# PJLab-ADG/neuralsim

Measured on AMD Instinct MI355X. Metric: training rays/sec (fwd+bwd) NeuS 800x800, higher is better.
Workload: dtype fp16

## Files before the change

### neuralsim_amd/csrc/field.hip

```cpp
#ifndef NSIM_SCATTER_SCAN_EXIT
#define NSIM_SCATTER_SCAN_EXIT 1
#endif
#include "lotd_dev.h"
#include "mfma_mlp.h"
#include "occ_dev.h"
#include <stdlib.h>

enum { M_W1 = 0, M_W2, M_W2T, M_W1T, M_R1, M_R2, M_R3, M_R3T, M_R2T, M_R1T, M_COUNT };
enum { V_B1 = 0, V_B2, V_WH, V_RB1, V_RB2, V_RB3, V_SCAL, V_COUNT };

struct FieldLayout {
  int64_t mat[M_COUNT];
  int64_t vec[V_COUNT];
  int64_t total;
  int elt;
  int split;
};

static const int kMatUo[M_COUNT] = {64, 64, 64, 32, 64, 64, 32, 64, 64, 32};
static const int kMatUi[M_COUNT] = {32, 64, 64, 64, 32, 64, 64, 32, 64, 64};

static inline int mat_uo(int m, int nc) { return m == M_W1T ? 32 * nc : kMatUo[m]; }
static inline int mat_ui(int m, int nc) { return m == M_W1 ? 32 * nc : kMatUi[m]; }
static inline int field_nc(int num_levels) { return num_levels > 16 ? 2 : 1; }
static inline int field_ne(const NsimFieldMeta* meta) { return meta->embed_E > 0 ? 2 : 0; }
static inline int field_ni(const NsimFieldMeta* meta) { return field_nc(meta->lotd.num_levels) + field_ne(meta); }

static inline FieldLayout field_layout(int precision, int nc = 1) {
  FieldLayout L;
  L.elt = precision == 0 ? 2 : 4;
  L.split = precision == 2 ? 1 : 0;
  int64_t off = 0;
  for (int m = 0; m < M_COUNT; ++m) {
    L.mat[m] = off;
    off += (int64_t)mat_uo(m, nc) * mat_ui(m, nc) * L.elt;
  }
  for (int v = 0; v < V_COUNT; ++v) {
    L.vec[v] = off;
    off += 64 * 4;
  }
  L.total = off;
  return L;
}

struct SrcOff {
  int w1, w2, wh, b1, b2, bh;
  int r1, r2, r3, rb1, rb2, rb3;
  int n_sdf_w, n_sdf_b, n_rad_w, n_rad_b;
};
__host__ __device__ inline SrcOff src_off(int D, int F1 = 32) {
  SrcOff o;
  o.w1 = 0;
  o.w2 = 64 * F1;
  o.wh = (D == 2) ? 64 * F1 + 4096 : 64 * F1;
  o.n_sdf_w = o.wh + 64;
  o.b1 = 0;
  o.b2 = 64;
  o.bh = (D == 2) ? 128 : 64;
  o.n_sdf_b = o.bh + 1;
  o.r1 = 0;
  o.r2 = 64 * 26;
  o.r3 = 64 * 26 + 4096;
  o.n_rad_w = o.r3 + 192;
  o.rb1 = 0;
  o.rb2 = 64;
  o.rb3 = 128;
  o.n_rad_b = 131;
  return o;
}


#define SPLIT_LO_SCALE 2048.0f
__device__ __forceinline__ float f16_sat(float v) { return fminf(fmaxf(v, -65504.0f), 65504.0f); }
__device__ __forceinline__ void split_f16(float v, f16& hi, f16& lo) {
  v = f16_sat(v);
  hi = (f16)v;
// ... 52 lines not shown
        ((f16*)(wpack + L.mat[m]))[k] = whi;
        if (L.split) ((f16*)(wpack + L.mat[m]))[cnt + k] = (f16)((w - (float)whi) * SPLIT_LO_SCALE);
      } else {
        const int lane = (int)(k & 63);
        const int fr = (int)(k >> 6);
        const int r = fr & 15, fm = fr >> 4;
        const int nMi = Ui / 32;
        const int mo = fm / nMi, mi = fm % nMi;
        row = 32 * mo + (lane & 31);
        col = unit_of(mi, r, lane >> 5);
        ((float*)(wpack + L.mat[m]))[k] = pack_src(m, row, col, D, F1, dims.E, dims.EB, sdf_w, rad_w);
      }
      return;
    }
    base += cnt;
  }
  const int64_t vtid = tid - base;
  if (vtid >= 0 && vtid < (int64_t)V_COUNT * 64) {
    const int v = (int)(vtid >> 6), k = (int)(vtid & 63);
    const int hi = k >> 5, m = (k >> 4) & 1, r = k & 15;
    const int u = unit_of(m, r, hi);
    const SrcOff o = src_off(D, F1 + dims.E);
    float val = 0.f;
    switch (v) {
      case V_B1: val = sdf_b[o.b1 + u]; break;
      case V_B2: val = D == 2 ? sdf_b[o.b2 + u] : 0.f; break;
      case V_WH: val = sdf_w[o.wh + u]; break;
      case V_RB1: val = rad_b[o.rb1 + u]; break;
      case V_RB2: val = rad_b[o.rb2 + u]; break;
      case V_RB3: val = (u < 3) ? rad_b[o.rb3 + u] : 0.f; break;
      case V_SCAL: val = (k == 0) ? sdf_b[o.bh] : 0.f; break;
    }
    ((float*)(wpack + L.vec[v]))[k] = val;
  }
}

__global__ void __launch_bounds__(256) k_field_pack(FieldLayout L, PackDims dims, int D, int F1, const float* __restrict__ sdf_w,
                                                     const float* __restrict__ sdf_b, const float* __restrict__ rad_w,
                                                     const float* __restrict__ rad_b, char* __restrict__ wpack) {
  field_pack_elem(L, dims, D, F1, sdf_w, sdf_b, rad_w, rad_b, wpack, (int64_t)blockIdx.x * blockDim.x + threadIdx.x);
}

struct PackTwo {
  FieldLayout L[2];
  PackDims dims[2];
  char* out[2];
};
__global__ void __launch_bounds__(256) k_field_pack2(PackTwo p, int D, int F1, const float* __restrict__ sdf_w,
                                                      const float* __restrict__ sdf_b, const float* __restrict__ rad_w,
                                                      const float* __restrict__ rad_b) {
  const int64_t tid = (int64_t)blockIdx.x * blockDim.x + threadIdx.x;
  if (blockIdx.y == 0) field_pack_elem(p.L[0], p.dims[0], D, F1, sdf_w, sdf_b, rad_w, rad_b, p.out[0], tid);
  else field_pack_elem(p.L[1], p.dims[1], D, F1, sdf_w, sdf_b, rad_w, rad_b, p.out[1], tid);
}

#define NSIM_LOG2E 1.4426950408889634f
#define NSIM_LN2 0.6931471805599453f
__device__ __forceinline__ float softplus_exact(float z, float beta, float inv_beta) {
  const float t = nsim_exp2(-fabsf(z) * (beta * NSIM_LOG2E));
  return fmaxf(z, 0.f) + nsim_log2(1.0f + t) * (inv_beta * NSIM_LN2);
}
#ifdef NSIM_PROBE_CHEAP_ACT
__device__ __forceinline__ float softplus_b(float z, float beta, float inv_beta) {
  const float q = fmaxf(0.f, 1.0f - 0.25f * beta * fabsf(z));
  return fmaxf(z, 0.f) + q * q * (inv_beta * NSIM_LN2);
}
// ... 128 lines not shown
__device__ long long g_ktime1[3][64 * 24];
__device__ long long g_kiter[3][64 * 32];
#define KT(K, i)                                                                                          \
  if (blockIdx.x < 64 && wave == 0 && lane == 0) {                                                        \
    if ((i) == 0 && grp >= 0 && (grp - (int64_t)blockIdx.x) / (int64_t)gridDim.x < 32)                    \
      g_kiter[K][blockIdx.x * 32 + (grp - (int64_t)blockIdx.x) / (int64_t)gridDim.x] =                   \
          (long long)__builtin_amdgcn_s_memtime();                                                        \
    if (grp == (int64_t)blockIdx.x + gridDim.x || (i) >= 20)                                              \
      g_ktime[K][blockIdx.x * 24 + (i)] = (long long)__builtin_amdgcn_s_memtime();                        \
    else if (grp == (int64_t)blockIdx.x)                                                                  \
      g_ktime1[K][blockIdx.x * 24 + (i)] = (long long)__builtin_amdgcn_s_memtime();                       \
  }
extern "C" int nsim_debug_ktime(long long* out) {
  return (int)hipMemcpyFromSymbol(out, HIP_SYMBOL(g_ktime), sizeof(g_ktime));
}
extern "C" int nsim_debug_kiter(long long* out) {
  return (int)hipMemcpyFromSymbol(out, HIP_SYMBOL(g_kiter), sizeof(g_kiter));
}
extern "C" int nsim_debug_ktime1(long long* out) {
  return (int)hipMemcpyFromSymbol(out, HIP_SYMBOL(g_ktime1), sizeof(g_ktime1));
}
#else
#define KT(K, i)
#endif

template <int PREC>
__device__ __forceinline__ const char* stage_weights(char* smem, const FieldArgs& a, int first, int count,
                                                     FieldLayout& Lk, int& lds_used) {
  Lk = a.lay;
  nsim_prefetch_own_code(a.code_pf, smem);
  if constexpr (PREC != 1) {
    const int64_t m0 = a.lay.mat[first];
    const int64_t m1 = (first + count < M_COUNT) ? a.lay.mat[first + count] : a.lay.vec[0];
    const int64_t mbytes = m1 - m0, vbytes = a.lay.total - a.lay.vec[0];
    const f16x8* src = reinterpret_cast<const f16x8*>(a.wpack + m0);
    f16x8* dst = reinterpret_cast<f16x8*>(smem);
    for (int i = threadIdx.x; i < (int)(mbytes >> 4); i += blockDim.x) dst[i] = src[i];
    const f16x8* vsrc = reinterpret_cast<const f16x8*>(a.wpack + a.lay.vec[0]);
    f16x8* vdst = reinterpret_cast<f16x8*>(smem + mbytes);
    for (int i = threadIdx.x; i < (int)(vbytes >> 4); i += blockDim.x) vdst[i] = vsrc[i];
    for (int m = 0; m < M_COUNT; ++m) Lk.mat[m] = a.lay.mat[m] - m0;
    for (int v = 0; v < V_COUNT; ++v) Lk.vec[v] = mbytes + (a.lay.vec[v] - a.lay.vec[0]);
    lds_used = (int)((mbytes + vbytes + 15) & ~15);
    __syncthreads();
    return smem;
  } else {
    lds_used = 0;
    return a.wpack;
  }
}

__device__ __forceinline__ float vecf(const char* W, const FieldLayout& L, int v, int hi, int k) {
  return reinterpret_cast<const float*>(W + L.vec[v])[hi * 32 + k];
}

struct alignas(8) nsim_f2 { float x, y; };
template <class T>
struct alignas(2 * sizeof(T)) JPair;
template <class T>
__device__ __forceinline__ void jload6(const T* p, float (&a)[3], float (&b)[3]);
template <class T>
struct alignas(2 * sizeof(T)) JPair {
  T x, y;
};
template <class T>
__device__ __forceinline__ void jstore6(T* p, const float (&a)[3], const float (&b)[3]) {
  JPair<T>* q = reinterpret_cast<JPair<T>*>(p);
// ... 1038 lines not shown
#pragma unroll
      for (int q = 0; q < 4; ++q)
#pragma unroll
        for (int b = 0; b < 2; ++b) {
          const int l = 16 * m + 4 * q + 2 * hi + b, r0 = 16 * m + 4 * q + 2 * b;
          if (!LV_OK(l)) continue;
          float* dp = a.dh_pl + ((int64_t)l * a.S + s) * 2;
          dp[0] = dh[r0];
          dp[1] = dh[r0 + 1];
        }
    }
    KT(1, 16);
    KT(1, 17);
  }
  { const int64_t grp = -1; KT(1, 21); }
  const int F1 = 2 * a.lotd.num_levels, FIN = F1 + (NE ? a.embed_E : 0);
  const SrcOff so = src_off(SDF_D, FIN);
  const int64_t ro = (int64_t)(blockIdx.x & (unsigned)a.rep_mask) * a.rep_stride;
  auto flush_w1 = [&](int mo, int no, const f32x16& acc) {
    if (no < NC) jflush_tile(a.dsdf_w + ro + so.w1, FIN, 64, F1, mo, no, acc);
    else jflush_tile(a.dsdf_w + ro + so.w1 + (F1 - 32 * NC), FIN, 64, 32 * NC + a.embed_E, mo, no, acc);
  };
#pragma unroll
  for (int q = 0; q < NPAIR; ++q) flush_w1(wave >> 1, 2 * q + (wave & 1), accW1[q]);
  if constexpr (NODD) flush_w1(wave & 1, NI - 1, accW1[NPAIR]);
  if constexpr (SDF_D == 2) {
    jflush_tile(a.dsdf_w + ro + so.w2, 64, 64, 64, wave >> 1, wave & 1, accW2);
    if (bs2 != 0.f) atomicAdd(&a.dsdf_b[ro + so.b2 + lane], bs2);
  }
  if (bs1 != 0.f) atomicAdd(&a.dsdf_b[ro + so.b1 + lane], bs1);
  if (bsh != 0.f) atomicAdd(&a.dsdf_w[ro + so.wh + lane], bsh);
  if (lane == 0 && bh != 0.f) atomicAdd(&a.dsdf_b[ro + so.bh], bh);
  { const int64_t grp = -1; KT(1, 22); }
}

#define SDF_H_SCALE 1024.0f
#ifndef NSIM_SDF_MIN_WAVES
#define NSIM_SDF_MIN_WAVES 2
#endif
#ifndef NSIM_SDF_NBUF
#define NSIM_SDF_NBUF 1
#endif
#ifndef GLM_PTS
#define GLM_PTS 2
#endif
#ifndef GLM_PTS_WJ
#define GLM_PTS_WJ 1
#endif
#ifndef NSIM_GATHER_WJ_WAVES
#define NSIM_GATHER_WJ_WAVES 1
#endif
#ifndef NSIM_GATHER_SLOTS_WJ
#define NSIM_GATHER_SLOTS_WJ 1
#endif
#ifndef NSIM_GATHER_SLOTS
#define NSIM_GATHER_SLOTS 0
#endif
template <int PREC, bool WJ>
__global__ void __launch_bounds__(64, WJ ? NSIM_GATHER_WJ_WAVES : 1) k_lotd_gather_lm(FieldArgs a) {
  using JT = typename JPlane<PREC>::T;
  constexpr int NP = WJ ? GLM_PTS_WJ : GLM_PTS;
  const int lane = nsim_lane();
  const int xcd = (int)(blockIdx.x & 7u);
  const int64_t s0 = (int64_t)(blockIdx.x >> 3) * (64 * NP) + lane;
  int64_t Sv = a.S;
  if (a.S_dev) {
// ... 822 lines not shown
        g_grad_scratch[i].floats >= (int64_t)R * n)
      return g_grad_scratch[i].buf;
  return nullptr;
}

static void grad_scratch_fold(float* sc, int R, int64_t n_w, int64_t n_b, float* dst_w, float* dst_b, hipStream_t stream) {
  const int64_t n = n_w + n_b;
  hipLaunchKernelGGL(k_rep_reduce, dim3(nsim_blocks(n, 256)), dim3(256), 0, stream, sc, R, n, n_w, dst_w, dst_b, n);
}

static FieldArgs field_args(const NsimFieldMeta* meta) {
  FieldArgs a = FieldArgs();
  a.lotd = lotd_dev(&meta->lotd);
  a.lay = field_layout(meta->precision, field_ni(meta));
  a.embed_E = meta->embed_E;
  a.beta = meta->softplus_beta > 0.f ? meta->softplus_beta : 1e30f;
  static const int code_pf = getenv("NSIM_CODE_PREFETCH") ? atoi(getenv("NSIM_CODE_PREFETCH")) : 0;
  a.code_pf = code_pf;
  return a;
}

static unsigned field_grid(int64_t S, int64_t max_blocks, int waves = FIELD_WAVES) {
  const int64_t tiles = (S + 31) / 32;
  int64_t b = (tiles + waves - 1) / waves;
  if (b > max_blocks) b = max_blocks;
  if (b < 1) b = 1;
  return (unsigned)b;
}

static size_t weights_lds_bytes(const NsimFieldMeta* meta, int first = 0, int count = M_COUNT) {
  if (meta->precision == 1) return 0;
  const FieldLayout L = field_layout(meta->precision, field_ni(meta));
  const int64_t m1 = (first + count < M_COUNT) ? L.mat[first + count] : L.vec[0];
  return (size_t)(((m1 - L.mat[first]) + (L.total - L.vec[0]) + 15) & ~15);
}
static size_t stage_bytes(const NsimFieldMeta* meta) {
  return meta->precision == 0 ? stage_bytes_per_wave<0>() : stage_bytes_per_wave<1>();
}

static int field_waves(const NsimFieldMeta* meta, int mode) {
  return (mode == 2 && meta->precision == 0 && field_nc(meta->lotd.num_levels) == 2) ? 3 : FIELD_WAVES;
}

template <int MODE>
static int field_launch(const NsimFieldMeta* meta, const FieldArgs& a, size_t shmem, int64_t max_blocks,
                        hipStream_t stream, bool gl2 = false) {
  const int nw = field_waves(meta, MODE);
  const dim3 grid(field_grid(a.S, max_blocks, nw)), block(64 * nw);
  const int key = meta->precision * 2 + (meta->sdf_D - 1);
  if (field_ne(meta)) {
    if constexpr (MODE == 3) {
      switch ((field_nc(meta->lotd.num_levels) - 1) * 4 + key) {
        case 0: hipLaunchKernelGGL((k_field<0, 1, 3, 1, false, 2>), grid, block, shmem, stream, a); break;
        case 1: hipLaunchKernelGGL((k_field<0, 2, 3, 1, false, 2>), grid, block, shmem, stream, a); break;
        case 2: hipLaunchKernelGGL((k_field<1, 1, 3, 1, false, 2>), grid, block, shmem, stream, a); break;
        case 3: hipLaunchKernelGGL((k_field<1, 2, 3, 1, false, 2>), grid, block, shmem, stream, a); break;
        case 4: hipLaunchKernelGGL((k_field<0, 1, 3, 2, false, 2>), grid, block, shmem, stream, a); break;
        case 5: hipLaunchKernelGGL((k_field<0, 2, 3, 2, false, 2>), grid, block, shmem, stream, a); break;
        case 6: hipLaunchKernelGGL((k_field<1, 1, 3, 2, false, 2>), grid, block, shmem, stream, a); break;
        case 7: hipLaunchKernelGGL((k_field<1, 2, 3, 2, false, 2>), grid, block, shmem, stream, a); break;
      }
      NSIM_CHECK_LAUNCH();
      return 0;
    } else {
      return 36;
    }
  }
// ... 29 lines not shown
  return 0;
}

static int bwd_ablate() {
  const char* ab = getenv("NSIM_ABLATE");
  return ab ? atoi(ab) : 0;
}

#define FIELD_GRID_FWD 1024
#define FIELD_GRID_BWD 256

extern "C" {

int64_t nsim_field_wpack_bytes(const NsimFieldMeta* meta) {
  if (field_meta_check(meta)) return -1;
  return field_layout(meta->precision, field_ni(meta)).total;
}

int nsim_field_pack_weights(const NsimFieldMeta* meta, const float* sdf_w, const float* sdf_b, const float* rad_w,
                            const float* rad_b, void* wpack, void* stream) {
  const int rc = field_meta_check(meta);
  if (rc) return rc;
  const int nc = field_ni(meta);
  const FieldLayout L = field_layout(meta->precision, nc);
  PackDims dims;
  dims.E = meta->embed_E;
  dims.EB = 32 * field_nc(meta->lotd.num_levels);
  int64_t total = 0;
  for (int m = 0; m < M_COUNT; ++m) {
    dims.uo[m] = mat_uo(m, nc);
    dims.ui[m] = mat_ui(m, nc);
    total += (int64_t)dims.uo[m] * dims.ui[m];
  }
  total += (int64_t)V_COUNT * 64;
  hipLaunchKernelGGL(k_field_pack, dim3(nsim_blocks(total, 256)), dim3(256), 0, (hipStream_t)stream, L, dims,
                     meta->sdf_D, 2 * meta->lotd.num_levels, sdf_w, sdf_b, rad_w, rad_b, (char*)wpack);
  NSIM_CHECK_LAUNCH();
  return 0;
}

int nsim_jplane_elem_bytes(const NsimFieldMeta* meta) { return meta ? NSIM_J_ELEM_BYTES(meta->precision) : 0; }

int nsim_field_pack_weights2(const NsimFieldMeta* meta_a, void* wpack_a, const NsimFieldMeta* meta_b, void* wpack_b,
                             const float* sdf_w, const float* sdf_b, const float* rad_w, const float* rad_b, void* stream) {
  int rc = field_meta_check(meta_a);
  if (rc) return rc;
  rc = field_meta_check(meta_b);
  if (rc) return rc;
  if (meta_a->sdf_D != meta_b->sdf_D || meta_a->lotd.num_levels != meta_b->lotd.num_levels || meta_a->embed_E != meta_b->embed_E) return 2;
  if (!wpack_a || !wpack_b) return 4;
  const int nc = field_ni(meta_a);
  PackTwo p;
  const NsimFieldMeta* ms[2] = {meta_a, meta_b};
  int64_t most = 0;
  for (int q = 0; q < 2; ++q) {
    p.L[q] = field_layout(ms[q]->precision, nc);
    int64_t total = (int64_t)V_COUNT * 64;
    p.dims[q].E = meta_a->embed_E;
    p.dims[q].EB = 32 * field_nc(meta_a->lotd.num_levels);
    for (int m = 0; m < M_COUNT; ++m) {
      p.dims[q].uo[m] = mat_uo(m, nc);
      p.dims[q].ui[m] = mat_ui(m, nc);
      total += (int64_t)p.dims[q].uo[m] * p.dims[q].ui[m];
    }
    most = total > most ? total : most;
  }
  p.out[0] = (char*)wpack_a;
  p.out[1] = (char*)wpack_b;
  hipLaunchKernelGGL(k_field_pack2, dim3(nsim_blocks(most, 256), 2), dim3(256), 0, (hipStream_t)stream, p, meta_a->sdf_D,
                     2 * meta_a->lotd.num_levels, sdf_w, sdf_b, rad_w, rad_b);
  NSIM_CHECK_LAUNCH();
  return 0;
}

static void deal_levels(const NsimFieldMeta* meta, FieldArgs& a) {
  const int NL = field_nc(meta->lotd.num_levels) == 2 ? ((meta->lotd.num_levels + 7) & ~7) : 16;
  float cost[32], load[8] = {0, 0, 0, 0, 0, 0, 0, 0}, total = 0.f;
  bool used[32] = {false};
  for (int l = 0; l < NL; ++l) {
    cost[l] = l >= meta->lotd.num_levels ? (NL > 16 ? 0.05f : 0.35f) : (meta->lotd.type[l] == NSIM_LOTD_HASH ? 1.0f : 0.35f);
    total += cost[l];
  }
  const float limit = total / 8.0f * 1.08f;
  for (int xc = 0; xc < 8; ++xc) a.glm_n[xc] = 0;
  auto least = [&]() {
    int tx = 0;
    for (int xc = 1; xc < 8; ++xc)
      if (load[xc] < load[tx]) tx = xc;
    return tx;
  };
  auto put = [&](int xc, int l, int half, float c) {
    a.glm_lv[xc][(int)a.glm_n[xc]] = (signed char)l;
    a.glm_half[xc][(int)a.glm_n[xc]++] = (signed char)half;
    load[xc] += c;
  };
  auto tsize = [&](int l) { return l < meta->lotd.num_levels ? meta->lotd.size[l] : 0u; };
  for (int it = 0; it < NL; ++it) {
// ... 241 lines not shown
struct BwdPos {
  const float *x, *rays_o, *rays_d, *t;
  const int64_t* ridx;
};
static int field_bwd_sdf(const NsimFieldMeta* meta, const void* wpack, const BwdPos* pos, const float* h_planes,
                         const void* J_planes, int64_t S, const float* dsdf, const float* gn, float* dh_planes, float* g_planes,
                         float* dsdf_w, float* dsdf_b, float* dx, int64_t plane_pitch, void* stream) {
  const int rc = field_meta_check_full(meta);
  if (rc) return rc;
  if (S <= 0) return 0;
  if (!dsdf_w || !dsdf_b) return 26;
  if (!h_planes || !J_planes) return 28;
  if ((dh_planes != nullptr) != (g_planes != nullptr)) return 28;
  const int ne = field_ne(meta);
  if ((ne != 0) != (pos != nullptr)) return 36;
  if (ne && dx) return 36;
  FieldArgs a = field_args(meta);
  a.wpack = (const char*)wpack;
  if (pos) {
    if (!pos->x && !(pos->rays_o && pos->rays_d && pos->t && pos->ridx)) return 24;
    a.x = pos->x; a.rays_o = pos->rays_o; a.rays_d = pos->rays_d; a.t = pos->t; a.ridx = pos->ridx;
  }
  a.S = S;
  if (plane_pitch != 0 && (plane_pitch < S || (plane_pitch & 31))) return 28;
  a.PS = plane_pitch ? plane_pitch : NSIM_PLANE_PITCH(S);
  a.dsdf = dsdf; a.dnablas = gn;
  a.h_pl = const_cast<float*>(h_planes); a.J_pl = const_cast<void*>(J_planes);
  a.dh_pl = dh_planes; a.g_pl = g_planes;
  a.dsdf_w = dsdf_w; a.dsdf_b = dsdf_b;
  a.dx = dx;
  a.ablate = bwd_ablate();
  const int nc = field_nc(meta->lotd.num_levels), nw = field_waves(meta, 2);
  const char* oldp = getenv("NSIM_SDF_BWD_OLD");
  if (ne || !(oldp && atoi(oldp) == 1)) {
    const size_t row = meta->precision == 0 ? jstage_row_bytes<0>() : jstage_row_bytes<1>();
    const int ni = nc + ne;
    const bool dbuf = NSIM_BWD_DBUF && meta->precision == 0 && !ne && (nc == 2 || NSIM_BWD_JDIRECT);
    const size_t shmem = weights_lds_bytes(meta, 0, 4) + (dbuf ? 2 : 1) * (128 + (ni > 2 ? 32 * ni : 64)) * row +
                         (meta->precision == 0 && nc == 1 && !ne ? (size_t)JOINT_WAVES * (NSIM_BWD_JDIRECT ? 4096 : 16384) : 0);
    const int64_t tiles = (S + 31) / 32;
    int64_t nb = (tiles + JOINT_WAVES - 1) / JOINT_WAVES;
    const char* gcap = getenv("NSIM_SDF_BWD_GRID");
    const int64_t cap = gcap ? atoi(gcap) : 256;
    nb = nb > cap ? cap : (nb < 1 ? 1 : nb);
    const dim3 grid((unsigned)nb), block(64 * JOINT_WAVES);
    const SrcOff so = src_off(meta->sdf_D, 2 * meta->lotd.num_levels + meta->embed_E);
    int R = 1;
    float* sc = nb >= grad_replicas_min_wg() ? grad_scratch(stream, so.n_sdf_w + so.n_sdf_b, R) : nullptr;
    if (sc) {
      a.dsdf_w = sc; a.dsdf_b = sc + so.n_sdf_w;
      a.rep_mask = R - 1; a.rep_stride = so.n_sdf_w + so.n_sdf_b;
    }
    switch ((ne ? 8 : 0) + (nc - 1) * 4 + meta->precision * 2 + (meta->sdf_D - 1)) {
      case 8: hipLaunchKernelGGL((k_field_bwd_j<0, 1, 1, 2>), grid, block, shmem, (hipStream_t)stream, a); break;
      case 9: hipLaunchKernelGGL((k_field_bwd_j<0, 2, 1, 2>), grid, block, shmem, (hipStream_t)stream, a); break;
      case 10: hipLaunchKernelGGL((k_field_bwd_j<1, 1, 1, 2>), grid, block, shmem, (hipStream_t)stream, a); break;
      case 11: hipLaunchKernelGGL((k_field_bwd_j<1, 2, 1, 2>), grid, block, shmem, (hipStream_t)stream, a); break;
      case 12: hipLaunchKernelGGL((k_field_bwd_j<0, 1, 2, 2>), grid, block, shmem, (hipStream_t)stream, a); break;
      case 13: hipLaunchKernelGGL((k_field_bwd_j<0, 2, 2, 2>), grid, block, shmem, (hipStream_t)stream, a); break;
      case 14: hipLaunchKernelGGL((k_field_bwd_j<1, 1, 2, 2>), grid, block, shmem, (hipStream_t)stream, a); break;
      case 15: hipLaunchKernelGGL((k_field_bwd_j<1, 2, 2, 2>), grid, block, shmem, (hipStream_t)stream, a); break;
      case 0: hipLaunchKernelGGL((k_field_bwd_j<0, 1>), grid, block, shmem, (hipStream_t)stream, a); break;
      case 1: hipLaunchKernelGGL((k_field_bwd_j<0, 2>), grid, block, shmem, (hipStream_t)stream, a); break;
      case 2: hipLaunchKernelGGL((k_field_bwd_j<1, 1>), grid, block, shmem, (hipStream_t)stream, a); break;
      case 3: hipLaunchKernelGGL((k_field_bwd_j<1, 2>), grid, block, shmem, (hipStream_t)stream, a); break;
      case 4: hipLaunchKernelGGL((k_field_bwd_j<0, 1, 2>), grid, block, shmem, (hipStream_t)stream, a); break;
      case 5: hipLaunchKernelGGL((k_field_bwd_j<0, 2, 2>), grid, block, shmem, (hipStream_t)stream, a); break;
// ... 112 lines not shown
```

### neuralsim_amd/csrc/mfma_mlp.h

```cpp
#pragma once
#include "nsim_common.h"

__device__ __forceinline__ int unit_of(int m, int r, int hi) { return 32 * m + (r & 3) + 8 * (r >> 2) + 4 * hi; }


__device__ __forceinline__ f32x16 zero16() {
  f32x16 z;
#pragma unroll
  for (int r = 0; r < 16; ++r) z[r] = 0.f;
  return z;
}

template <int PREC, int N>
__device__ __forceinline__ float dyn_scale(const float (&v)[N]) {
  if constexpr (PREC == 1) {
    return 1.0f;
  } else {
    float m = 0.f;
#pragma unroll
    for (int i = 0; i < N; ++i) m = fmaxf(m, fabsf(v[i]));
    m = wave_max(m);
    if (!(m > 0.f) || !(m < 3.0e38f)) return 1.0f;
    uint32_t bits;
    memcpy(&bits, &m, 4);
// ... 288 lines not shown
      for (int q = 0; q < 32; ++q) s += a[lane * P + 32 * wave + q];
    }
  }
  return s;
}

__device__ __forceinline__ void jflush_tile(float* dst, int ld, int rows, int cols, int mo, int no, const f32x16& acc) {
  const int lane = nsim_lane(), col = 32 * no + (lane & 31), hi = lane >> 5;
  if (col >= cols) return;
#pragma unroll
  for (int r = 0; r < 16; ++r) {
    const int row = 32 * mo + mfma_row(r, hi);
    if (row < rows && acc[r] != 0.f) atomicAdd(&dst[row * ld + col], acc[r]);
  }
}

__device__ __forceinline__ bool halfwave_run_sum2(int64_t key, bool valid, float& v0, float& v1) {
  const int lane = nsim_lane();
  const int64_t k = valid ? key : (int64_t)-1 - lane;
  const int64_t pk = wave_shfl(k, lane - 1);
  const unsigned long long heads = wave_ballot((lane & 31) == 0 || pk != k);
  const unsigned long long below = heads & ((2ull << lane) - 1ull);
  const int run_start = 63 - __builtin_clzll(below);
#pragma unroll
  for (int d = 1; d < 32; d <<= 1) {
    const float o0 = wave_shfl(v0, lane - d), o1 = wave_shfl(v1, lane - d);
    if (lane - d >= run_start) {
      v0 += o0;
      v1 += o1;
    }
  }
  return valid && ((lane & 31) == 31 || ((heads >> (lane + 1)) & 1ull));
}
```

Baseline: 6.911 million.

## Add 16-point-tile SDF backward kernel using 16x16x32 MFMA and packed fp16 weights

Adds a second fp16 weight layout pre-swizzled for 16x16x32 MFMA operands and a new joint SDF backward kernel that processes 16-point tiles per wave instead of 32. Weight gradients use bf16 LDS staging with transposed LDS reads (ds_read_tr16), and hash-plane values are prefetched asynchronously into LDS. The kernel runs by default for fp16, single-chunk, no-embedding configs and raises the grid cap. In exchange it adds more staging syncs per tile and a larger packed weight buffer.

```diff
diff --git a/neuralsim_amd/csrc/field.hip b/neuralsim_amd/csrc/field.hip
--- a/neuralsim_amd/csrc/field.hip
+++ b/neuralsim_amd/csrc/field.hip
@@ -12,6 +12,8 @@
 struct FieldLayout {
   int64_t mat[M_COUNT];
   int64_t vec[V_COUNT];
+  int64_t vend;
+  int64_t mat16[4];
   int64_t total;
   int elt;
   int split;
@@ -39,9 +41,15 @@
     L.vec[v] = off;
     off += 64 * 4;
   }
+  L.vend = off;
+  for (int m = 0; m < 4; ++m) {
+    L.mat16[m] = off;
+    if (precision == 0 && nc == 1) off += (int64_t)mat_uo(m, 1) * mat_ui(m, 1) * 2;
+  }
   L.total = off;
   return L;
 }
+__host__ __device__ inline bool field_has16(const FieldLayout& L) { return L.total > L.vend; }
 
 struct SrcOff {
   int w1, w2, wh, b1, b2, bh;
@@ -160,6 +168,21 @@
       case V_SCAL: val = (k == 0) ? sdf_b[o.bh] : 0.f; break;
     }
     ((float*)(wpack + L.vec[v]))[k] = val;
+    return;
+  }
+  int64_t t16 = vtid - (int64_t)V_COUNT * 64;
+  if (!field_has16(L) || t16 < 0) return;
+  for (int m = 0; m < 4; ++m) {
+    const int Uo = dims.uo[m], Ui = dims.ui[m];
+    const int64_t cnt = (int64_t)Uo * Ui;
+    if (t16 < cnt) {
+      const int e = (int)(t16 & 7), lane = (int)((t16 >> 3) & 63), fs = (int)(t16 >> 9);
+      const int nS = Ui / 32, mo = fs / nS, c = fs % nS;
+      const int row = 16 * mo + (lane & 15), col = 32 * c + 16 * (e >> 2) + 4 * (lane >> 4) + (e & 3);
+      ((f16*)(wpack + L.mat16[m]))[t16] = (f16)pack_src(m, row, col, D, F1, dims.E, dims.EB, sdf_w, rad_w);
+      return;
+    }
+    t16 -= cnt;
   }
 }
 
@@ -354,7 +377,7 @@
   if constexpr (PREC != 1) {
     const int64_t m0 = a.lay.mat[first];
     const int64_t m1 = (first + count < M_COUNT) ? a.lay.mat[first + count] : a.lay.vec[0];
-    const int64_t mbytes = m1 - m0, vbytes = a.lay.total - a.lay.vec[0];
+    const int64_t mbytes = m1 - m0, vbytes = a.lay.vend - a.lay.vec[0];
     const f16x8* src = reinterpret_cast<const f16x8*>(a.wpack + m0);
     f16x8* dst = reinterpret_cast<f16x8*>(smem);
     for (int i = threadIdx.x; i < (int)(mbytes >> 4); i += blockDim.x) dst[i] = src[i];
@@ -1459,6 +1482,277 @@
   if (bsh != 0.f) atomicAdd(&a.dsdf_w[ro + so.wh + lane], bsh);
   if (lane == 0 && bh != 0.f) atomicAdd(&a.dsdf_b[ro + so.bh], bh);
   { const int64_t grp = -1; KT(1, 22); }
+}
+
+__device__ __forceinline__ const char* stage_weights16(char* smem, const FieldArgs& a, FieldLayout& Lk, int& lds_used) {
+  Lk = a.lay;
+  nsim_prefetch_own_code(a.code_pf, smem);
+  const int64_t m0 = a.lay.mat16[0], mbytes = a.lay.total - m0, vbytes = a.lay.vend - a.lay.vec[0];
+  const f16x8* src = reinterpret_cast<const f16x8*>(a.wpack + m0);
+  f16x8* dst = reinterpret_cast<f16x8*>(smem);
+  for (int i = threadIdx.x; i < (int)(mbytes >> 4); i += blockDim.x) dst[i] = src[i];
+  const f16x8* vsrc = reinterpret_cast<const f16x8*>(a.wpack + a.lay.vec[0]);
+  f16x8* vdst = reinterpret_cast<f16x8*>(smem + mbytes);
+  for (int i = threadIdx.x; i < (int)(vbytes >> 4); i += blockDim.x) vdst[i] = vsrc[i];
+  for (int m = 0; m < 4; ++m) Lk.mat16[m] = a.lay.mat16[m] - m0;
+  for (int v = 0; v < V_COUNT; ++v) Lk.vec[v] = mbytes + (a.lay.vec[v] - a.lay.vec[0]);
+  lds_used = (int)((mbytes + vbytes + 15) & ~15);
+  __syncthreads();
+  return smem;
+}
+static size_t weights16_lds_bytes(const FieldLayout& L) { return (size_t)(((L.total - L.mat16[0]) + (L.vend - L.vec[0]) + 15) & ~15); }
+
+__device__ __forceinline__ float vec16(const char* W, const FieldLayout& L, int v, int vb, int k) {
+  return reinterpret_cast<const float*>(W + L.vec[v])[vb + 16 * (k >> 3) + 8 * ((k >> 2) & 1) + (k & 3)];
+}
+
+#define BWD16_PF_BYTES 2048
+
+template <int SDF_D>
+__global__ void __launch_bounds__(64 * JOINT_WAVES, 2) k_field_bwd_h(FieldArgs a) {
+  using JT = typename JPlane<0>::T;
+  NSIM_DYN_SMEM(smem);
+  const int lane = nsim_lane(), p = lane & 15, g = lane >> 4;
+  const int wave = (int)(threadIdx.x >> 6);
+  const float beta = a.beta, inv_beta = 1.0f / a.beta;
+  FieldLayout L;
+  int wbytes = 0;
+  const char* W = stage_weights16(smem, a, L, wbytes);
+  char* const stA = smem + wbytes;
+  char* const stB = stA + J16_STAGE_BYTES;
+  char* const stC = stB + J16_STAGE_BYTES;
+  char* const pf = stC + J16_STAGE_BYTES + wave * BWD16_PF_BYTES;
+  const int vb = 32 * (g & 1) + 4 * (g >> 1);
+  f32x4 accW1[2], accW2[4];
+#pragma unroll
+  for (int n = 0; n < 2; ++n) accW1[n] = zero4();
+#pragma unroll
+  for (int n = 0; n < 4; ++n) accW2[n] = zero4();
+  float bs1 = 0.f, bs2 = 0.f, bsh = 0.f, bh = 0.f;
+  const bool do_dw = !(a.ablate & 4);
+
+  const int64_t ntiles = (a.S + 15) / 16;
+  const int64_t ngroups = (ntiles + JOINT_WAVES - 1) / JOINT_WAVES;
+  auto prefetch_planes = [&](int64_t tile_n) {
+    const int64_t s0 = tile_n * 16;
+#pragma unroll
+    for (int i = 0; i < 2; ++i)
+      nsim_glds16(a.h_pl + ((int64_t)(8 * i + (lane >> 3)) * a.PS + s0) * 2 + 4 * (lane & 7), pf + 1024 * i);
+  };
+  {
+    const int64_t t0 = (int64_t)blockIdx.x * JOINT_WAVES + wave;
+    if (t0 < ntiles) prefetch_planes(t0);
+  }
+  for (int64_t grp = blockIdx.x; grp < ngroups; grp += gridDim.x) {
+    const int64_t s = (grp * JOINT_WAVES + wave) * 16 + p;
+    const bool valid = s < a.S;
+    const int vo = nsim_opaque_zero();
+    const char* Wv = W + vo;
+    float gs = 0.f, gn[3] = {0.f, 0.f, 0.f};
+    float h[8];
+    JPair<JT> Jq[4][3];
+    nsim_wait_vm0();
+    const int64_t sc = valid ? s : a.S - 1;
+#pragma unroll
+    for (int m = 0; m < 2; ++m)
+#pragma unroll
+      for (int b = 0; b < 2; ++b) {
+        const int l = 8 * m + 2 * g + b, r0 = 4 * m + 2 * b;
+        const float* hp = reinterpret_cast<const float*>(pf + 128 * l) + 2 * p;
+        h[r0] = valid ? hp[0] : 0.f;
+        h[r0 + 1] = valid ? hp[1] : 0.f;
+      }
+    nsim_wait_lgkm0();
+    if (valid) {
+      if (a.dsdf) gs = a.dsdf[s];
+      if (a.dnablas) {
+#pragma unroll
+        for (int c = 0; c < 3; ++c) gn[c] = a.dnablas[3 * s + c];
+      }
+    }
+#pragma unroll
+    for (int m = 0; m < 2; ++m)
+#pragma unroll
+      for (int b = 0; b < 2; ++b) {
+        const int l = 8 * m + 2 * g + b;
+        const JPair<JT>* jp = reinterpret_cast<const JPair<JT>*>(reinterpret_cast<const JT*>(a.J_pl) + ((int64_t)l * a.PS + sc) * 6);
+        Jq[2 * m + b][0] = jp[0];
+        Jq[2 * m + b][1] = jp[1];
+        Jq[2 * m + b][2] = jp[2];
+      }
+    {
+      const int64_t tn = (grp + gridDim.x) * JOINT_WAVES + wave;
+      if (tn < ntiles) prefetch_planes(tn);
+    }
+    float a1[16];
+    dense16<4, 2>(a1, W + L.mat16[M_W1], h, true);
+#pragma unroll
+    for (int k = 0; k < 16; ++k) a1[k] = softplus_b(a1[k] + vec16(Wv, L, V_B1, vb, k), beta, inv_beta);
+    float a2[16];
+    float d1[16];
+    if constexpr (SDF_D == 2) {
+      dense16<4, 4>(a2, W + L.mat16[M_W2], a1, false);
+#pragma unroll
+      for (int k = 0; k < 16; ++k) a2[k] = softplus_b(a2[k] + vec16(Wv, L, V_B2, vb, k), beta, inv_beta);
+      float d2[16];
+#pragma unroll
+      for (int k = 0; k < 16; ++k) d2[k] = sig_from_softplus(a2[k], beta) * vec16(Wv, L, V_WH, vb, k);
+      dense16<4, 4>(d1, W + L.mat16[M_W2T], d2, false);
+#pragma unroll
+      for (int k = 0; k < 16; ++k) d1[k] = sig_from_softplus(a1[k], beta) * d1[k];
+    } else {
+#pragma unroll
+      for (int k = 0; k < 16; ++k) {
+        a2[k] = a1[k];
+        d1[k] = sig_from_softplus(a1[k], beta) * vec16(Wv, L, V_WH, vb, k);
+      }
+    }
+    {
+      float gg[8];
+      dense16<2, 4>(gg, W + L.mat16[M_W1T], d1, false);
+      if (valid && a.g_pl) {
+#pragma unroll
+        for (int m = 0; m < 2; ++m)
+#pragma unroll
+          for (int b = 0; b < 2; ++b) {
+            const int l = 8 * m + 2 * g + b, r0 = 4 * m + 2 * b;
+            float* gp = a.g_pl + ((int64_t)l * a.S + s) * 2;
+            gp[0] = gg[r0];
+            gp[1] = gg[r0 + 1];
+          }
+      }
+    }
+    float gh[8];
+#pragma unroll
+    for (int e = 0; e < 4; ++e) {
+      const int r0 = 4 * (e >> 1) + 2 * (e & 1);
+      const float mk = valid ? 1.f : 0.f;
+      gh[r0] = mk * ((float)Jq[e][0].x * gn[0] + (float)Jq[e][0].y * gn[1] + (float)Jq[e][1].x * gn[2]);
+      gh[r0 + 1] = mk * ((float)Jq[e][1].y * gn[0] + (float)Jq[e][2].x * gn[1] + (float)Jq[e][2].y * gn[2]);
+    }
+    __syncthreads();
+    jstage16<4>(stA, d1, wave);
+    jstage16<2>(stB, gh, wave);
+    __syncthreads();
+    if (do_dw) jdw16_tiles<2>(stA, wave, stB, 0, accW1, nullptr);
+    float dh1[16];
+    dense16<4, 2>(dh1, W + L.mat16[M_W1], gh, true);
+    float dz1[16], whv[16];
+    if constexpr (SDF_D == 2) {
+      float eh1[16];
+#pragma unroll
+      for (int k = 0; k < 16; ++k) {
+        const float s1 = sig_from_softplus(a1[k], beta);
+        dz1[k] = dh1[k] * d1[k] * (beta * (1.0f - s1));
+        eh1[k] = dh1[k] * s1;
+      }
+      float d2[16];
+#pragma unroll
+      for (int k = 0; k < 16; ++k) d2[k] = sig_from_softplus(a2[k], beta) * vec16(Wv, L, V_WH, vb, k);
+      __syncthreads();
+      jstage16<4>(stA, d2, wave);
+      jstage16<4>(stB, eh1, wave);
+      __syncthreads();
+      if (do_dw) jdw16_tiles<4>(stA, wave, stB, 0, accW2, nullptr);
+      float dh2[16];
+      dense16<4, 4>(dh2, W + L.mat16[M_W2], eh1, true);
+      float dz2[16];
+#pragma unroll
+      for (int k = 0; k < 16; ++k) {
+        const float s2 = sig_from_softplus(a2[k], beta);
+        const float wh = vec16(Wv, L, V_WH, vb, k);
+        whv[k] = dh2[k] * s2 + gs * a2[k];
+        dz2[k] = gs * wh * s2 + dh2[k] * wh * (beta * s2 * (1.0f - s2));
+      }
+      __syncthreads();
+      jstage16<4>(stA, dz2, wave);
+      jstage16<4>(stB, a1, wave);
+      jstage16<4>(stC, whv, wave);
+      __syncthreads();
+      if (do_dw) {
+        jdw16_tiles<4>(stA, wave, stB, 0, accW2, &bs2);
+        bsh += j16_row_share(stC, wave);
+      }
+      float da1[16];
+      dense16<4, 4>(da1, W + L.mat16[M_W2T], dz2, true);
+#pragma unroll
+      for (int k = 0; k < 16; ++k) dz1[k] = dz1[k] + da1[k] * sig_from_softplus(a1[k], beta);
+    } else {
+#pragma unroll
+      for (int k = 0; k < 16; ++k) {
+        const float s1 = sig_from_softplus(a1[k], beta);
+        const float wh = vec16(Wv, L, V_WH, vb, k);
+        whv[k] = dh1[k] * s1 + gs * a1[k];
+        dz1[k] = gs * wh * s1 + dh1[k] * wh * (beta * s1 * (1.0f - s1));
+      }
+    }
+    bh += wave_sum(g == 0 ? gs : 0.f);
+    __syncthreads();
+    jstage16<4>(stA, dz1, wave);
+    jstage16<2>(stB, h, wave);
+    if constexpr (SDF_D == 1) jstage16<4>(stC, whv, wave);
+    __syncthreads();
+    if (do_dw) {
+      jdw16_tiles<2>(stA, wave, stB, 0, accW1, &bs1);
+      if constexpr (SDF_D == 1) bsh += j16_row_share(stC, wave);
+    }
+    float dh[8];
+    dense16<2, 4>(dh, W + L.mat16[M_W1T], dz1, true);
+    if (a.dx) {
+      float acc[3] = {0.f, 0.f, 0.f};
+      if (valid) {
+#pragma unroll
+        for (int m = 0; m < 2; ++m)
+#pragma unroll
+          for (int b = 0; b < 2; ++b) {
+            const int l = 8 * m + 2 * g + b, r0 = 4 * m + 2 * b;
+            float ja[3], jb[3];
+            jload6(reinterpret_cast<const JT*>(a.J_pl) + ((int64_t)l * a.PS + s) * 6, ja, jb);
+#pragma unroll
+            for (int c3 = 0; c3 < 3; ++c3) acc[c3] = acc[c3] + dh[r0] * ja[c3] + dh[r0 + 1] * jb[c3];
+          }
+      }
+#pragma unroll
+      for (int c3 = 0; c3 < 3; ++c3) {
+        acc[c3] = acc[c3] + wave_shfl_xor(acc[c3], 16);
+        acc[c3] = acc[c3] + wave_shfl_xor(acc[c3], 32);
+      }
+      if (valid && g == 0) {
+#pragma unroll
+        for (int c3 = 0; c3 < 3; ++c3) a.dx[3 * s + c3] = a.dx[3 * s + c3] + acc[c3];
+      }
+    }
+    if (valid && a.dh_pl) {
+#pragma unroll
+      for (int m = 0; m < 2; ++m)
+#pragma unroll
+        for (int b = 0; b < 2; ++b) {
+          const int l = 8 * m + 2 * g + b, r0 = 4 * m + 2 * b;
+          float* dp = a.dh_pl + ((int64_t)l * a.S + s) * 2;
+          dp[0] = dh[r0];
+          dp[1] = dh[r0 + 1];
+        }
+    }
+  }
+  const int F1 = 2 * a.lotd.num_levels;
+  const SrcOff so = src_off(SDF_D, F1);
+  const int64_t ro = (int64_t)(blockIdx.x & (unsigned)a.rep_mask) * a.rep_stride;
+#pragma unroll
+  for (int n = 0; n < 2; ++n) jflush16(a.dsdf_w + ro + so.w1, F1, F1, wave, n, accW1[n]);
+  bs1 += wave_shfl_xor(bs1, 16);
+  bs1 += wave_shfl_xor(bs1, 32);
+  bsh += wave_shfl_xor(bsh, 16);
+  bsh += wave_shfl_xor(bsh, 32);
+  if constexpr (SDF_D == 2) {
+#pragma unroll
+    for (int n = 0; n < 4; ++n) jflush16(a.dsdf_w + ro + so.w2, 64, 64, wave, n, accW2[n]);
+    bs2 += wave_shfl_xor(bs2, 16);
+    bs2 += wave_shfl_xor(bs2, 32);
+    if (g == 0 && bs2 != 0.f) atomicAdd(&a.dsdf_b[ro + so.b2 + 16 * wave + p], bs2);
+  }
+  if (g == 0 && bs1 != 0.f) atomicAdd(&a.dsdf_b[ro + so.b1 + 16 * wave + p], bs1);
+  if (g == 0 && bsh != 0.f) atomicAdd(&a.dsdf_w[ro + so.wh + 16 * wave + p], bsh);
+  if (lane == 0 && bh != 0.f) atomicAdd(&a.dsdf_b[ro + so.bh], bh);
 }
 
 #define SDF_H_SCALE 1024.0f
@@ -2347,7 +2641,7 @@
   if (meta->precision == 1) return 0;
   const FieldLayout L = field_layout(meta->precision, field_ni(meta));
   const int64_t m1 = (first + count < M_COUNT) ? L.mat[first + count] : L.vec[0];
-  return (size_t)(((m1 - L.mat[first]) + (L.total - L.vec[0]) + 15) & ~15);
+  return (size_t)(((m1 - L.mat[first]) + (L.vend - L.vec[0]) + 15) & ~15);
 }
 static size_t stage_bytes(const NsimFieldMeta* meta) {
   return meta->precision == 0 ? stage_bytes_per_wave<0>() : stage_bytes_per_wave<1>();
@@ -2443,7 +2737,7 @@
     dims.ui[m] = mat_ui(m, nc);
     total += (int64_t)dims.uo[m] * dims.ui[m];
   }
-  total += (int64_t)V_COUNT * 64;
+  total += (int64_t)V_COUNT * 64 + (L.total - L.vend) / 2;
   hipLaunchKernelGGL(k_field_pack, dim3(nsim_blocks(total, 256)), dim3(256), 0, (hipStream_t)stream, L, dims,
                      meta->sdf_D, 2 * meta->lotd.num_levels, sdf_w, sdf_b, rad_w, rad_b, (char*)wpack);
   NSIM_CHECK_LAUNCH();
@@ -2474,6 +2768,7 @@
       p.dims[q].ui[m] = mat_ui(m, nc);
       total += (int64_t)p.dims[q].uo[m] * p.dims[q].ui[m];
     }
+    total += (p.L[q].total - p.L[q].vend) / 2;
     most = total > most ? total : most;
   }
   p.out[0] = (char*)wpack_a;
@@ -2781,7 +3076,30 @@
   a.ablate = bwd_ablate();
   const int nc = field_nc(meta->lotd.num_levels), nw = field_waves(meta, 2);
   const char* oldp = getenv("NSIM_SDF_BWD_OLD");
-  if (ne || !(oldp && atoi(oldp) == 1)) {
+  const bool old_kernel = oldp && atoi(oldp) == 1;
+  const char* tile_env = getenv("NSIM_BWD_TILE");
+  if (!old_kernel && meta->precision == 0 && nc == 1 && !ne && field_has16(a.lay) && !(tile_env && atoi(tile_env) == 32)) {
+    const size_t shmem = weights16_lds_bytes(a.lay) + 3 * J16_STAGE_BYTES + JOINT_WAVES * BWD16_PF_BYTES;
+    const int64_t tiles = (S + 15) / 16;
+    int64_t nb = (tiles + JOINT_WAVES - 1) / JOINT_WAVES;
+    const char* gcap = getenv("NSIM_SDF_BWD_GRID");
+    const int64_t cap = gcap ? atoi(gcap) : 512;
+    nb = nb > cap ? cap : (nb < 1 ? 1 : nb);
+    const dim3 grid((unsigned)nb), block(64 * JOINT_WAVES);
+    const SrcOff so = src_off(meta->sdf_D, 2 * meta->lotd.num_levels);
+    int R = 1;
+    float* sc = nb >= grad_replicas_min_wg() ? grad_scratch(stream, so.n_sdf_w + so.n_sdf_b, R) : nullptr;
+    if (sc) {
+      a.dsdf_w = sc; a.dsdf_b = sc + so.n_sdf_w;
+      a.rep_mask = R - 1; a.rep_stride = so.n_sdf_w + so.n_sdf_b;
+    }
+    if (meta->sdf_D == 1) hipLaunchKernelGGL((k_field_bwd_h<1>), grid, block, shmem, (hipStream_t)stream, a);
+    else hipLaunchKernelGGL((k_field_bwd_h<2>), grid, block, shmem, (hipStream_t)stream, a);
+    if (sc) grad_scratch_fold(sc, R, so.n_sdf_w, so.n_sdf_b, dsdf_w, dsdf_b, (hipStream_t)stream);
+    NSIM_CHECK_LAUNCH();
+    return 0;
+  }
+  if (ne || !old_kernel) {
     const size_t row = meta->precision == 0 ? jstage_row_bytes<0>() : jstage_row_bytes<1>();
     const int ni = nc + ne;
     const bool dbuf = NSIM_BWD_DBUF && meta->precision == 0 && !ne && (nc == 2 || NSIM_BWD_JDIRECT);
diff --git a/neuralsim_amd/csrc/mfma_mlp.h b/neuralsim_amd/csrc/mfma_mlp.h
--- a/neuralsim_amd/csrc/mfma_mlp.h
+++ b/neuralsim_amd/csrc/mfma_mlp.h
@@ -344,3 +344,150 @@
   }
   return valid && ((lane & 31) == 31 || ((heads >> (lane + 1)) & 1ull));
 }
+
+
+typedef float f32x4 __attribute__((ext_vector_type(4)));
+typedef __bf16 bf16x4 __attribute__((ext_vector_type(4)));
+
+__device__ __forceinline__ f32x4 zero4() {
+  f32x4 z;
+#pragma unroll
+  for (int r = 0; r < 4; ++r) z[r] = 0.f;
+  return z;
+}
+
+#if defined(__HIP__)
+__device__ __forceinline__ f32x4 mfma_16x16x32_f16(f16x8 a, f16x8 b, f32x4 c) {
+  return __builtin_amdgcn_mfma_f32_16x16x32_f16(a, b, c, 0, 0, 0);
+}
+__device__ __forceinline__ f32x4 mfma_16x16x32_bf16(bf16x8 a, bf16x8 b, f32x4 c) {
+  return __builtin_amdgcn_mfma_f32_16x16x32_bf16(a, b, c, 0, 0, 0);
+}
+#else
+template <class V>
+inline f32x4 mfma_16x16x32_portable(V a, V b, f32x4 c) {
+  const int lane = nsim_lane(), col = lane & 15, g = lane >> 4;
+  f32x4 d = c;
+  for (int G = 0; G < 4; ++G) {
+    const V bs = wave_shfl(b, 16 * G + col);
+    for (int r = 0; r < 4; ++r) {
+      const V as = wave_shfl(a, 16 * G + 4 * g + r);
+      float s = 0.f;
+      for (int e = 0; e < 8; ++e) s += (float)as[e] * (float)bs[e];
+      d[r] += s;
+    }
+  }
+  return d;
+}
+inline f32x4 mfma_16x16x32_f16(f16x8 a, f16x8 b, f32x4 c) { return mfma_16x16x32_portable(a, b, c); }
+inline f32x4 mfma_16x16x32_bf16(bf16x8 a, bf16x8 b, f32x4 c) { return mfma_16x16x32_portable(a, b, c); }
+#endif
+
+__device__ __forceinline__ bf16x4 lds_read_tr16(const bf16* p) {
+#if defined(__HIP__)
+  return __builtin_amdgcn_ds_read_tr16_b64_v4bf16((__attribute__((address_space(3))) bf16x4*)p);
+#else
+  const int lane = nsim_lane(), G = lane >> 4, i = lane & 15;
+  const unsigned long long me = (unsigned long long)(uintptr_t)p;
+  bf16x4 r;
+  for (int q = 0; q < 4; ++q) {
+    const unsigned long long src = wave_shfl(me, 16 * G + 4 * q + (i >> 2));
+    r[q] = reinterpret_cast<const bf16*>((uintptr_t)src)[i & 3];
+  }
+  return r;
+#endif
+}
+
+template <int MO, int NT>
+__device__ __forceinline__ void contract16(f32x4 (&acc)[MO], const char* wmat, const float (&in)[NT * 4], float in_scale) {
+  static_assert(NT % 2 == 0, "contract16: whole K-steps of 32 inputs");
+  const int lane = nsim_lane();
+  const f16x8* A = reinterpret_cast<const f16x8*>(wmat);
+#pragma unroll
+  for (int c = 0; c < NT / 2; ++c) {
+    f16x8 b;
+#pragma unroll
+    for (int e = 0; e < 8; ++e) b[e] = (f16)(in[8 * c + e] * in_scale);
+#pragma unroll
+    for (int mo = 0; mo < MO; ++mo) acc[mo] = mfma_16x16x32_f16(A[(mo * (NT / 2) + c) * 64 + lane], b, acc[mo]);
+  }
+}
+
+template <int MO, int NT>
+__device__ __forceinline__ void dense16(float (&out)[MO * 4], const char* wmat, const float (&in)[NT * 4], bool dynamic) {
+  f32x4 acc[MO];
+#pragma unroll
+  for (int mo = 0; mo < MO; ++mo) acc[mo] = zero4();
+  const float sc = dynamic ? dyn_scale<0, NT * 4>(in) : 1.0f;
+  contract16<MO, NT>(acc, wmat, in, sc);
+  const float inv = 1.0f / sc;
+#pragma unroll
+  for (int mo = 0; mo < MO; ++mo)
+#pragma unroll
+    for (int r = 0; r < 4; ++r) out[mo * 4 + r] = acc[mo][r] * inv;
+}
+
+#define J16_PTS (16 * JOINT_WAVES)
+#define J16_ROW 128
+#define J16_STAGE_BYTES (J16_PTS * J16_ROW)
+
+__device__ __forceinline__ int j16_swz(int row) { return (((row >> 1) & 3) << 2) | (row & 1) | ((row >> 2) & 2); }
+
+template <int NT>
+__device__ __forceinline__ void jstage16(void* st, const float (&v)[NT * 4], int wave) {
+  const int lane = nsim_lane(), p = lane & 15, g = lane >> 4;
+  const int row = 16 * wave + p;
+  char* base = reinterpret_cast<char*>(st) + row * J16_ROW;
+  const int swz = j16_swz(row);
+#pragma unroll
+  for (int m = 0; m < NT; ++m) {
+    bf16x4 w;
+    bf16 b0, b1, b2, b3;
+    nsim_cvt2_bf16(v[4 * m], v[4 * m + 1], b0, b1);
+    nsim_cvt2_bf16(v[4 * m + 2], v[4 * m + 3], b2, b3);
+    w[0] = b0; w[1] = b1; w[2] = b2; w[3] = b3;
+    *reinterpret_cast<bf16x4*>(base + 8 * ((4 * m + g) ^ swz)) = w;
+  }
+}
+
+__device__ __forceinline__ bf16x8 j16_operand(const void* st, int t, int c) {
+  const int lane = nsim_lane(), G = lane >> 4, q = (lane >> 2) & 3, pc = lane & 3;
+  const char* base = reinterpret_cast<const char*>(st);
+  bf16x8 o;
+#pragma unroll
+  for (int h = 0; h < 2; ++h) {
+    const int row = 32 * c + 16 * h + 4 * G + q;
+    const bf16x4 v = lds_read_tr16(reinterpret_cast<const bf16*>(base + row * J16_ROW + 8 * ((4 * t + pc) ^ j16_swz(row))));
+#pragma unroll
+    for (int e = 0; e < 4; ++e) o[4 * h + e] = v[e];
+  }
+  return o;
+}
+
+template <int NB>
+__device__ __forceinline__ void jdw16_tiles(const void* stA, int ta, const void* stB, int tb0, f32x4 (&acc)[NB], float* rs) {
+#pragma unroll
+  for (int c = 0; c < J16_PTS / 32; ++c) {
+    const bf16x8 av = j16_operand(stA, ta, c);
+    if (rs) *rs = nsim_bf16x8_sum(av, *rs);
+#pragma unroll
+    for (int n = 0; n < NB; ++n) acc[n] = mfma_16x16x32_bf16(av, j16_operand(stB, tb0 + n, c), acc[n]);
+  }
+}
+
+__device__ __forceinline__ float j16_row_share(const void* st, int t) {
+  float s = 0.f;
+#pragma unroll
+  for (int c = 0; c < J16_PTS / 32; ++c) s = nsim_bf16x8_sum(j16_operand(st, t, c), s);
+  return s;
+}
+
+__device__ __forceinline__ void jflush16(float* dst, int ld, int cols, int to, int tn, const f32x4& acc) {
+  const int lane = nsim_lane(), col = 16 * tn + (lane & 15);
+  if (col >= cols) return;
+#pragma unroll
+  for (int r = 0; r < 4; ++r) {
+    const int row = 16 * to + 4 * (lane >> 4) + r;
+    if (acc[r] != 0.f) atomicAdd(&dst[row * ld + col], acc[r]);
+  }
+}
```

Result: faster. 7.127 million, median of 6 (+3.1%).
